# kabachuha/sd-webui-text2video

Measured on AMD Instinct MI355X. Metric: denoised frames/sec (UNet+VAE), ModelScope 24f@256x256, higher is better.
Workload: dtype f16; 1 GPU; ModelScope t2v fp16 (random-init 1.41B UNetSD + VAE decoder), 24 frames @ 256x256, 50 DDIM_Gaussian steps, CFG 9.0 (BASELINE.json configs[1]); one step = one whole video; frames_per_video=24, videos_per_batch=1, layout=single, layout_requested=auto, parallelism=1 GPU: cond+uncond batched as b=2

## Files before the change

include/t2v_hip.h:

```cpp
#ifndef T2V_HIP_H
#define T2V_HIP_H

#include <stdint.h>

#ifdef __cplusplus
extern "C" {
#endif

#define T2V_ABI_VERSION 11

#define T2V_OK 0
#define T2V_ERR_BAD_ARG (-1)
#define T2V_ERR_UNSUPPORTED (-2)
#define T2V_ERR_LAUNCH (-3)
#define T2V_ERR_NO_DEVICE (-4)
#define T2V_ERR_COMM (-5)
#define T2V_ERR_ASYNC (-6)
#define T2V_ERR_RESIDENCY (-7)

#define T2V_RELPOS_MAX_FRAMES 1024
#define T2V_RELPOS_LONG_PADL 72
#define T2V_RELPOS_LONG_COLS(R) ((2 * (R) + 158) / 8 * 8)

enum t2v_op_kind {
// ... 26 lines not shown
enum t2v_gather {
  T2V_GATHER_PLAIN = 0,
  T2V_GATHER_CONV3X3 = 1,
  T2V_GATHER_TCONV3 = 2,
  T2V_GATHER_CONV3X3_C8 = 3
};

#define T2V_EPI_NONE 0
#define T2V_EPI_GEGLU 1
#define T2V_EPI_TATTN 2

#define T2V_EPI_STATS 3

#define T2V_EPI_GN 4
#define T2V_EPI_XATTN 5
#define T2V_GN_PIECES 36

#define T2V_F16 0
#define T2V_F32 1

#define T2V_EXT_SLOTS 16
#define T2V_EXT_X 1
#define T2V_EXT_T 2
#define T2V_EXT_CTX 3
#define T2V_EXT_OUT 4
#define T2V_EXT_XT 5
#define T2V_EXT_XT_OUT 6
#define T2V_EXT_NOISE 7
#define T2V_EXT_EPS 8
#define T2V_EXT_ADAPTER 9
// ... 60 lines not shown
```

sd-webui-text2video_amd/_lib.py:

```python
from __future__ import annotations

import ctypes
import os

_HERE = os.path.dirname(os.path.abspath(__file__))
LIB_PATH = os.environ.get("T2V_LIB_PATH") or os.path.join(_HERE, "libt2v_hip.so")

EXPERIMENTAL = os.environ.get("T2V_EXPERIMENTAL", "0") == "1"


def knob(name: str, default):
    if os.environ.get("T2V_EXPERIMENTAL", "0") == "1":
        return os.environ.get(name, default)
    return default


ABI_VERSION = 11
RELPOS_MAX_FRAMES = 1024
RELPOS_LONG_PADL = 72
OP_GEMM, OP_GROUPNORM, OP_LAYERNORM, OP_ATTENTION, OP_SOFTMAX = 1, 2, 3, 4, 5
OP_NCTHW_TO_CL, OP_CL_TO_NCTHW, OP_TIME_EMBED, OP_COPY2D, OP_DDIM_STEP, OP_MEMSET = 6, 7, 8, 9, 10, 11
OP_LINCOMB = 12
OP_RELPOS_ATTN = 13
OP_EMBED_ROWS = 14
OP_TO_UINT8, OP_ALLGATHER, OP_HALO_EXCHANGE = 15, 16, 17
OP_RESHARD_ROWS, OP_ALLTOALL, OP_STATS_HALO = 18, 19, 20
OP_RESAMPLE = 21
OP_DEPTH_TOKENS, OP_AVGPOOL2 = 22, 23
ACT_NONE, ACT_SILU, ACT_RELU = 0, 1, 2
GATHER_PLAIN, GATHER_CONV3X3, GATHER_TCONV3, GATHER_CONV3X3_C8 = 0, 1, 2, 3
EPI_NONE, EPI_GEGLU, EPI_TATTN, EPI_STATS, EPI_GN, EPI_XATTN = 0, 1, 2, 3, 4, 5
GN_PIECES = 36
F16, F32 = 0, 1
EXT_SLOTS = 16
EXT_X, EXT_T, EXT_CTX, EXT_OUT, EXT_XT, EXT_XT_OUT, EXT_NOISE, EXT_EPS = 1, 2, 3, 4, 5, 6, 7, 8
EXT_ADAPTER = 9
OP_NI, OP_NF, OP_NP = 32, 8, 12
GN_ROWS_PER_BLOCK = 64
SYNC_INTS = 4096
SYNC_BARRIER_INTS = 512
GN_PART_BYTES = 2 << 20

EXPORTS = [
    "t2v_abi_version", "t2v_last_error", "t2v_device_info", "t2v_run_ops", "t2v_plan_create",
    "t2v_plan_num_ops", "t2v_plan_run", "t2v_plan_run_timed", "t2v_plan_destroy",
    "t2v_unet_forward", "t2v_vae_decode", "t2v_ddim_step",
# ... 93 lines not shown
```

sd-webui-text2video_amd/csrc/executor.hip:

```cpp
#include <hip/hip_runtime.h>

#include <cstdio>
#include <cstring>
#include <string>
#include <vector>

#include "t2v_kernels.h"

namespace {

thread_local std::string g_err;

int fail(int code, const std::string& msg) {
  g_err = msg;
  return code;
}

struct Resolved {
  t2v_op op;
};

inline bool resolve_ptrs(t2v_op& op, const uint64_t* ext, int n_ext) {
  for (int k = 0; k < T2V_OP_NP; ++k) {
    const uint64_t v = op.p[k];
// ... 24 lines not shown
      } else if (g == T2V_GATHER_CONV3X3_C8) {
        if (op.i[10] != 8 || K != 72 || op.i[3] != 8) return bad("C8 conv needs Cin == lda == 8, K == 72");
      } else if (g != T2V_GATHER_PLAIN) {
        return bad("unknown gather mode");
      }
      if (g == T2V_GATHER_CONV3X3 || g == T2V_GATHER_CONV3X3_C8) {
        if (op.i[11] != 1 && op.i[11] != 2) return bad("stride must be 1 or 2");
        if (op.i[12] != 0 && op.i[12] != 1) return bad("upsample must be 0 or 1");
        if (op.i[13] <= 0 || op.i[14] <= 0 || M % (op.i[13] * op.i[14]) != 0) return bad("M not a multiple of Hout*Wout");
      }
      if (g == T2V_GATHER_TCONV3 && (op.i[8] <= 0 || op.i[9] <= 0 || M % (op.i[8] * op.i[9]) != 0))
        return bad("M not a multiple of F*HW");
      if (op.i[16] == T2V_EPI_GEGLU && (N % 32 != 0 || op.i[17] != T2V_F16)) return bad("GEGLU needs N % 32 == 0, fp16 out");
      if (op.i[16] == T2V_EPI_STATS && (op.p[7] == 0 || op.i[19] > 1 || (g == T2V_GATHER_PLAIN && op.i[8] == 1)))
        return bad("column statistics (T2V_EPI_STATS): strips pointer p[7], no split-K, no fused LayerNorm");
      if (op.i[16] < 0 || op.i[16] > T2V_EPI_XATTN) return bad("unknown epilogue");
      if (op.i[18] < 0 || op.i[18] > 2) return bad("unknown activation (0 none, 1 SiLU, 2 ReLU)");
      if (op.i[30] != 0) {
        if (op.i[30] < 0 || M > 2 * op.i[30] || op.p[4] == 0) return bad("residual row wrap i[30]: positive, M <= 2 * wrap, and a residual");
        if (op.i[16] == T2V_EPI_GEGLU || op.i[16] == T2V_EPI_TATTN || op.i[16] == T2V_EPI_XATTN || (g == T2V_GATHER_PLAIN && (op.i[12] != 0 || op.i[8] != 0)))
          return bad("residual row wrap i[30]: plain / statistics / GroupNorm epilogues only, not beside i[12] or a fused LayerNorm");
      }
      if (op.i[16] == T2V_EPI_XATTN) {
        const int tile = op.i[22];
        if (g != T2V_GATHER_PLAIN || N % 64 != 0 || K % 64 != 0 || op.i[17] != T2V_F16 || op.i[19] > 1 || op.i[18] != 0 || op.i[8] != 0 || op.i[11] == 1)
          return bad("fused cross-attention: plain gather, N = 64 * heads, K % 64 == 0, fp16 out, no split-K / activation / LayerNorm / hi + lo output");
        if (!(((tile == 8 || tile == 11) && N == 320) || ((tile == 0 || tile == 5) && N % 128 == 0))) return bad("fused cross-attention: tile 8 / 11 with N == 320, or tile 0 / 5 with N % 128 == 0");
        if (op.p[2] != 0 || op.p[3] != 0 || op.p[4] != 0 || op.p[8] == 0 || op.p[9] == 0 || !(op.f[1] > 0.f)) return bad("fused cross-attention: no bias / row bias / residual; K, V^T and a positive scale are required");
        if (op.i[25] < 1 || op.i[25] > 96 || op.i[24] < N || op.i[24] % 8 != 0 || op.i[26] < ((op.i[25] + 31) / 32) * 32 || op.i[26] % 8 != 0 || op.i[15] <= 0 || op.i[15] % 32 != 0 || op.i[27] < 0 || op.i[28] < 0)
          return bad("fused cross-attention: 1 .. 96 keys, ld(K) >= N, V^T rows of >= ceil32(keys) halfs, rows per sample a multiple of 32");
        if (op.i[5] < N || op.i[5] % 4 != 0) return bad("fused cross-attention: ldc");
        if (op.i[12] != 0) return bad("fused cross-attention: no residual wrap");
        return 0;
      }
      if (op.i[16] == T2V_EPI_GN) {
        const int tile = op.i[22], rows = op.i[24], groups = op.i[28];
        const int bm = tile == 8 ? 192 : 128, bn = (tile == 8 || tile == 11) ? 320 : (tile == 3 ? 256 : 128);
        if (g == T2V_GATHER_CONV3X3_C8 || (g == T2V_GATHER_CONV3X3 && op.i[12] != 0)) return bad("fused GroupNorm: not for the C8 stem / the upsampling gather");
        if (op.i[20] != 0 || K % 64 != 0 || op.i[18] != 0) return bad("fused GroupNorm: no bias along M, no activation, K % 64 == 0");
        if (g == T2V_GATHER_PLAIN && (op.i[8] != 0 || op.i[11] == 1)) return bad("fused GroupNorm: no fused LayerNorm / hi + lo output on the same op");
        if (groups <= 0 || N % groups != 0 || rows <= 0 || M % rows != 0) return bad("fused GroupNorm: N % groups == 0, rows per instance must divide M");
        if (op.i[19] > 1) {
          if (groups > 32 || N % 8 != 0 || N / 8 > 512 || op.p[6] == 0) return bad("fused GroupNorm on a split-K GEMM: groups <= 32, N % 8 == 0, N <= 4096, a slab workspace");
        } else {
          if (tile != 8 && tile != 11 && tile != 3 && tile != 5 && tile != 0) return bad("fused GroupNorm: tile must be 8, 11, 3, 5 or 0");
          if (tile == 0 && N % 128 != 0) return bad("fused GroupNorm on the 128x128-class kernel: N % 128 == 0");
          if (N / groups > bn || (bn + N / groups - 1) / (N / groups) + 1 > T2V_GN_PIECES) return bad("fused GroupNorm: a group no wider than the tile");
// ... 237 lines not shown
      p.res = reinterpret_cast<const float*>(op.p[4]);
      p.out = reinterpret_cast<void*>(op.p[5]);
      p.ws = reinterpret_cast<float*>(op.p[6]);
      p.halo = op.i[23];
      p.out_lo = (p.gather == T2V_GATHER_PLAIN && op.i[11] == 1) ? 1 : 0;
      if (p.gather == T2V_GATHER_PLAIN && op.i[16] != T2V_EPI_TATTN) { p.res_wrap = op.i[12]; p.a_wrap = op.i[13]; }
      if (op.i[30] > 0) p.res_wrap = op.i[30];
      const int tile = op.i[22];
      if (p.epi == T2V_EPI_TATTN) {
        p.F = op.i[8]; p.HW = op.i[9]; p.tpix = op.i[10];
        p.tiles_ps = (p.HW + p.tpix - 1) / p.tpix;
        p.attn_scale_log2 = op.f[1] * 1.44269504088896340736f;
        p.Hin = p.Win = 0; p.Cin = 0;
        return t2v_launch_gemm2(p, tile, s);
      }
      if (p.epi == T2V_EPI_XATTN) {
        p.epi = T2V_EPI_NONE;
        p.xa_k = reinterpret_cast<const f16*>(op.p[8]);
        p.xa_vt = reinterpret_cast<const f16*>(op.p[9]);
        p.xa_ldk = op.i[24]; p.xa_lc = op.i[25]; p.xa_lcp = op.i[26]; p.xa_k_sample = op.i[27]; p.xa_vt_sample = op.i[28];
        p.attn_scale_log2 = op.f[1] * 1.44269504088896340736f;
      }
      const bool ln_any = p.gather == T2V_GATHER_PLAIN && (op.i[8] == 1 || op.i[8] == 2);
      if (p.splitk > 1 && !ln_any) p.tickets = reinterpret_cast<int*>(op.p[7]);
      if (ln_any) {
        p.ln_gb = reinterpret_cast<const float*>(op.p[3]);
        p.rowbias = nullptr;
        p.ln_out = reinterpret_cast<f16*>(op.p[7]);
        p.ld_ln = op.i[9];
        p.ln_eps = op.f[0];
// ... 260 lines not shown
```

sd-webui-text2video_amd/csrc/gemm2.hip:

```cpp
#include "t2v_kernels.h"

namespace {

__device__ __attribute__((aligned(256))) unsigned char g2_zero_page[256];

constexpr int G_CONV_UP = 100;
constexpr int BM_OF(int wm, int tm) { return wm * tm * 32; }

template <int N>
__device__ __forceinline__ void wait_vmcnt() {
  asm volatile("s_waitcnt vmcnt(%0)" ::"n"(N) : "memory");
}

template <int WM, int WN, int TM, int TN, int BK, int STAGES, int MINW, int GATHER, int XE = 0, bool TAT = false>
__global__ __launch_bounds__(WM * WN * 64, MINW) void gemm2_kernel(const GemmParams p) {
  constexpr int NW = WM * WN;
  constexpr int BM = WM * TM * 32, BN = WN * TN * 32;
  constexpr int ROW_BYTES = BK * 2;
  constexpr int RPS = 1024 / ROW_BYTES;
  constexpr int CPR = BK / 8;
  constexpr int XSLABS = BM / RPS, WSLABS = BN / RPS;
  static_assert(XSLABS % NW == 0, "token slabs must divide evenly over the waves");
  constexpr int XPW = XSLABS / NW;
  constexpr int WPW = (WSLABS + NW - 1) / NW;
// ... 485 lines not shown
      else e = launch_cfg_gather<WM, WN, TM, TN, BK, STAGES, MINW, T2V_GATHER_CONV3X3>(p, s);
      break;
    case T2V_GATHER_TCONV3:
      if constexpr (GN_TILE) {
        if (gn_here) { e = launch_cfg_gather<WM, WN, TM, TN, BK, STAGES, MINW, T2V_GATHER_TCONV3, 2>(p, s); break; }
      }
      e = launch_cfg_gather<WM, WN, TM, TN, BK, STAGES, MINW, T2V_GATHER_TCONV3>(p, s);
      break;
    default: return hipErrorInvalidValue;
  }
  if (e != hipSuccess) return e;
  if (p.splitk > 1 && p.tickets == nullptr) e = p.gn_out != nullptr ? t2v_launch_splitk_reduce_gn(p, s) : t2v_launch_splitk_reduce(p, s);
  return e;
}

}

hipError_t t2v_launch_gemm2(const GemmParams& p, int tile, hipStream_t s) {
  switch (tile) {
    case 1: return launch_cfg<2, 4, 4, 2, 64, 2, 2>(p, s);
    case 2: return launch_cfg<4, 2, 2, 5, 64, 2, 2>(p, s);
    case 3: return launch_cfg<2, 4, 2, 2, 64, 3, 2>(p, s);
    case 4: return launch_cfg<2, 2, 2, 2, 64, 4, 1>(p, s);
    case 5: return launch_cfg<2, 4, 2, 1, 64, 4, 2>(p, s);
    case 8: return launch_cfg<6, 2, 1, 5, 64, 2, 3>(p, s);
    case 9: return launch_cfg<6, 2, 1, 4, 64, 2, 3>(p, s);
    case 10: return launch_cfg<6, 2, 1, 3, 64, 2, 3>(p, s);
    case 12: return launch_cfg<2, 2, 1, 1, 64, 4, 2>(p, s);
    case 11: return launch_cfg<4, 2, 1, 5, 64, 2, 2>(p, s);
    default: return hipErrorInvalidValue;
// ... 3 lines not shown
```

sd-webui-text2video_amd/csrc/t2v_kernels.h:

```cpp
#pragma once
#include <hip/hip_runtime.h>
#include <stdint.h>

#include <string>

#include "../../include/t2v_hip.h"

typedef _Float16 f16;
typedef f16 f16x4 __attribute__((ext_vector_type(4)));
typedef f16 f16x8 __attribute__((ext_vector_type(8)));
typedef float f32x4 __attribute__((ext_vector_type(4)));
typedef float f32x8 __attribute__((ext_vector_type(8)));
typedef float f32x16 __attribute__((ext_vector_type(16)));

struct GemmParams {
  const f16* A;
  const f16* W;
  const float* bias;
  const float* rowbias;
  const float* res;
  void* out;
  float* ws;
  int M, N, K;
  int m_begin;
// ... 16 lines not shown
  int out_lo;
  float* stats;
  int a_wrap, res_wrap;
  const float* gn_gb;
  f16* gn_out;
  double* gn_part;
  unsigned* gn_bar;
  unsigned* gn_fault;
  int ld_gn, gn_rows, gn_cpg, gn_silu, gn_lo, gn_store_out;
  float gn_eps;
  int ln_x;
  unsigned gn_seq, gn_want;
  const f16* xa_k;
  const f16* xa_vt;
  int xa_ldk, xa_lc, xa_lcp, xa_k_sample, xa_vt_sample;
};


#if defined(__HIP_DEVICE_COMPILE__) && !defined(__gfx950__) && !defined(__gfx942__)
#error "libt2v_hip is written for gfx950 (MI355X); the device-scope exchange helpers assume gfx94x / gfx950 memory semantics"
#endif

__device__ __forceinline__ void t2v_st_dev(float* p, f32x4 v) { asm volatile("global_store_dwordx4 %0, %1, off sc1" ::"v"(p), "v"(v) : "memory"); }
__device__ __forceinline__ f32x4 t2v_ld_dev(const float* p) {
  f32x4 v;
  asm volatile("global_load_dwordx4 %0, %1, off sc1" : "=&v"(v) : "v"(p) : "memory");
  return v;
}
__device__ __forceinline__ void t2v_wait_dev(f32x4& a, f32x4& b, f32x4& c, f32x4& d) {
  asm volatile("s_waitcnt vmcnt(0)" : "+v"(a), "+v"(b), "+v"(c), "+v"(d)::"memory");
// ... 93 lines not shown
  return hipSuccess;
}
inline long t2v_lcm(long a, long b) { long x = a, y = b; while (y) { const long t = x % y; x = y; y = t; } return a / x * b; }

inline void t2v_normalize_splitk(GemmParams& p, int bk, long tiles) {
  const int KT = (p.K + bk - 1) / bk;
  if (p.splitk > KT) p.splitk = KT;
  if (p.splitk < 1) p.splitk = 1;
  p.kt_per_split = (KT + p.splitk - 1) / p.splitk;
  p.splitk = (KT + p.kt_per_split - 1) / p.kt_per_split;
  if (p.splitk <= 1 || p.epi != T2V_EPI_NONE || tiles > T2V_SYNC_INTS || p.gn_out != nullptr) p.tickets = nullptr;
}

hipError_t t2v_launch_gemm(const GemmParams& p, hipStream_t s);
hipError_t t2v_launch_gemm2(const GemmParams& p, int tile, hipStream_t s);
hipError_t t2v_launch_splitk_reduce(const GemmParams& p, hipStream_t s);
hipError_t t2v_launch_splitk_reduce_gn(const GemmParams& p, hipStream_t s);
hipError_t t2v_launch_groupnorm(const t2v_op& op, hipStream_t s);
hipError_t t2v_launch_layernorm(const t2v_op& op, hipStream_t s);
hipError_t t2v_launch_attention(const t2v_op& op, hipStream_t s);
hipError_t t2v_launch_relpos_attention(const t2v_op& op, hipStream_t s);
hipError_t t2v_launch_softmax(const t2v_op& op, hipStream_t s);
hipError_t t2v_launch_ncthw_to_cl(const t2v_op& op, hipStream_t s);
hipError_t t2v_launch_cl_to_ncthw(const t2v_op& op, hipStream_t s);
hipError_t t2v_launch_to_uint8(const t2v_op& op, hipStream_t s);
hipError_t t2v_launch_resample(const t2v_op& op, hipStream_t s);
hipError_t t2v_launch_depth_tokens(const t2v_op& op, hipStream_t s);
hipError_t t2v_launch_avgpool2(const t2v_op& op, hipStream_t s);
hipError_t t2v_launch_reshard_rows(const t2v_op& op, hipStream_t s);
hipError_t t2v_launch_time_embed(const t2v_op& op, hipStream_t s);
// ... 889 lines not shown
```

sd-webui-text2video_amd/lowering.py:

```python
from __future__ import annotations

from typing import Callable, Dict, List, Optional, Tuple

import torch

from . import _lib as L
from . import packing as pk
from .program import Buf, Program, Ref, TShardSpec


class _Declarations:
    def __init__(self, label: str, keep_taps: bool = False):
        self.P = Program(label)
        self.P.keep_taps = keep_taps
        self.packer = pk.WeightPacker()

    def w_linear(self, key) -> Ref:
        return Ref("weight", 0, self.packer.add(key + ":lin", "f16", lambda sd, k=key: pk.pad_rows(pk.linear(sd[k + ".weight"]))))

    def conv3_kernel(self, key) -> Tuple[Callable, str]:
        return (lambda sd, k=key: sd[k + ".weight"]), ":c3"

    def w_conv3(self, key, cin_pad=0, form="") -> Ref:
        kernel, suffix = self.conv3_kernel(key)
# ... 23 lines not shown
        self.sharing = bool(getattr(net, "_share_now", False)) and B == 2 and x_batch == 1 and self.shard is None
        self.Bc = 1 if self.sharing else B
        self.x_dt, self.out_dt, self.ctx_dt = x_dt, out_dt, ctx_dt
        self.x_batch = x_batch if 0 < x_batch < B else 0
        self.precise = bool(getattr(net, "precise_operands", False))
        level = getattr(net, "precise_operands", False)
        self.precise_gn = self.precise and level != "r3"
        self.precise_ff = self.precise and level != "r3"
        self.precise_all_levels = level == "all"
        self.precise_attn = self.precise and bool(getattr(net, "precise_attn_out", False))
        self.precise_rs = self.precise and bool(getattr(net, "precise_resample", False))
        self.gn_strips = bool(getattr(net, "gn_producer_stats", False))
        self.last_stats: Optional[Buf] = None
        self.stem_dup = False
        self.P.small_rank_tiles = self.shard is not None
        prefixes = tuple(getattr(net, "split_weight_prefixes", ()) or ())
        if prefixes:
            self.P.weight_lo = lambda ref: (Ref("weight", 0, self.packer.add_lo(ref.name))
                                            if ref.name.startswith(prefixes) and ref.name.rsplit(":", 1)[-1] in ("lin", "lin2", "c3", "c3d", "t3", "qkv", "kv")
                                            else None)
        self.emb_slices: Dict[str, Tuple[int, int]] = {}
        self.kv_slices: Dict[str, Tuple[int, int]] = {}
        self.kv_all: Optional[Buf] = None

    def precise_at(self, flag: bool, h: int, w: int) -> bool:
        return bool(flag) and (self.precise_all_levels or (h == self.H and w == self.W))

    def w_proj(self, key, copies: int) -> Ref:
        assert copies in (1, 2)
        return self.w_linear(key) if copies == 1 else self.w_linear_dup(key)

# ... 150 lines not shown
        if parting:
            self.sharing, self.Bc = False, self.B
        a = P.alloc(self.Bc * F * hw, out_cols or inner, "f16")
        lo = a.ld
        if q is None and not self.to_q_attention(attn, nrm, a, inner, heads, hw, scale, shared_rows):
            q = P.alloc(Mq, inner, "f16")
            P.gemm(attn + ".to_q", nrm, self.w_linear(attn + ".to_q"), inner, inner, q)
        if q is not None:
            P.attention(attn, q.ref, kbuf.ref, vbuf.ref, a.ref, out_buf=a, nq=hw, nk=Lc, heads=heads,
                        b_outer=self.Bc, b_inner=F, q_strides=(inner, q_b_stride, hw * inner),
                        kv_strides=(kv.ld, Lc * kv.ld, 0), o_strides=(lo, F * hw * lo, hw * lo), scale=scale, **attn_kw)
            P.free(q)
        P.free(nrm)
        return a, shared_rows

    def ff_tail(self, tb, n: Buf, x3: Buf, inner, h, w) -> Buf:
        P, M = self.P, n.rows
        wg, bg = self.w_geglu(f"{tb}.ff.net.0.proj")
        g = P.alloc(M, 4 * inner, "f16")
        P.gemm(f"{tb}.ff.geglu", n, wg, 8 * inner, inner, g, bias=bg, epi=L.EPI_GEGLU)
        P.free(n)
        hilo = self.precise_at(self.precise_ff, h, w)
        x4 = P.alloc(M, 2 * inner if hilo else inner, "f16")
        P.gemm(f"{tb}.ff.net.2", g, self.w_linear(f"{tb}.ff.net.2"), inner, 4 * inner, x4.col_slice(0, inner) if hilo else x4,
               bias=self.vec(f"{tb}.ff.net.2.bias"), residual=x3, out_lo=hilo)
        P.free(g, x3)
        return x4

    def resample(self, prefix, attr, x: Buf, c, h, w, *, up, dest: Optional[Buf] = None, **conv_kw) -> Buf:
        hilo = bool(self.precise_rs and c % 64 == 0)
        x16 = self.operand16(prefix + ".cast", x, c, hilo)
        out = self.conv3(f"{prefix}.{attr}", x16, f"{prefix}.{attr}", c, h, w, stride=1 if up else 2, up=1 if up else 0, dest=dest, hilo=hilo,
                         **conv_kw)
# ... 141 lines not shown
```

sd-webui-text2video_amd/program.py:

```python
from __future__ import annotations

import ctypes
import math
import os
from dataclasses import dataclass, field
from typing import Dict, List, Optional, Tuple

from . import _lib as L

_ITEM = {"f16": 2, "f32": 4, "f64": 8, "u8": 1}
COLLECTIVE_KINDS = (L.OP_ALLGATHER, L.OP_HALO_EXCHANGE, L.OP_ALLTOALL, L.OP_STATS_HALO)
_DT = {"f16": L.F16, "f32": L.F32}


@dataclass(frozen=True)
class TShardSpec:
    size: int
    index: int
    counts: Tuple[int, ...]

    @staticmethod
    def make(total_frames: int, size: int, index: int) -> "TShardSpec":
        base = -(-total_frames // size)
        last = total_frames - base * (size - 1)
# ... 78 lines not shown
                    self.free_list[idx] = (off + n, size - n)
                self.live[off] = n
                return off
        if self.free_list and self.free_list[-1][0] + self.free_list[-1][1] == self.top:
            off, size = self.free_list.pop()
            self.top = off
        off = self.top
        self.top += n
        self.high = max(self.high, self.top)
        self.live[off] = n
        return off

    def free(self, off: int):
        n = self.live.pop(off)
        self.free_list.append((off, n))
        self.free_list.sort()
        merged: List[Tuple[int, int]] = []
        for o, s in self.free_list:
            if merged and merged[-1][0] + merged[-1][1] == o:
                merged[-1] = (merged[-1][0], merged[-1][1] + s)
            else:
                merged.append((o, s))
        self.free_list = merged


@dataclass
class Op:
    kind: int
    name: str
    i: List[int] = field(default_factory=lambda: [0] * L.OP_NI)
    f: List[float] = field(default_factory=lambda: [0.0] * L.OP_NF)
    p: List[Ref] = field(default_factory=lambda: [NULL] * L.OP_NP)
    flops: float = 0.0
    meta: dict = field(default_factory=dict)
    out: Optional["Buf"] = None
    out2: Optional["Buf"] = None


# ... 9 lines not shown
        self.small_rank_tiles = False
        self.gn_fused_slice_bytes = int(L.knob("T2V_GN_FUSED_SLICE", 64 * 1024))
        self.gn_fused_total_bytes = int(L.knob("T2V_GN_FUSED_TOTAL", 128 * 1024 * 1024))
        self.weight_lo = None
        self._sync: Buf = self.alloc(L.SYNC_INTS + L.SYNC_BARRIER_INTS, 1, "f32")
        self.splitk_tickets = L.knob("T2V_SPLITK_TICKETS", "0") != "0"
        self.gn_coop = os.environ.get("T2V_GN_COOP", "1") != "0"
        self.gn_epilogue = self.gn_coop and os.environ.get("T2V_GN_EPI", "1") != "0" and not L.exchange_disabled()
        self._gn_part: Optional[Buf] = self.alloc(L.GN_PART_BYTES, 1, "u8") if self.gn_epilogue else None
        self._deferred: List[Buf] = []

    def alloc(self, rows: int, cols: int, dtype: str, ld: Optional[int] = None) -> Buf:
        ld = cols if ld is None else ld
        off = self.arena.alloc(rows * ld * _ITEM[dtype])
        return Buf(Ref("arena", off), rows, cols, ld, dtype, off)

    def free(self, *bufs: Buf):
        for b in bufs:
            if b is None or b.alloc_off < 0 or not b.owns:
                continue
            if self.keep_taps and any(t.alloc_off == b.alloc_off for t in self.taps.values()):
                continue
            if self._is_operand_of_last_gemm(b):
                self._deferred.append(b)
                continue
            self.arena.free(b.alloc_off)

    def _is_operand_of_last_gemm(self, b: Buf) -> bool:
        if not getattr(self, "gn_epilogue", False) or not self.ops:
            return False
# ... 267 lines not shown
                       stats=int(with_stats))
        if ln_fused:
            op.out2 = ln[3]
        if step_invariant:
            op.meta["step_invariant"] = True
        self._emit(op)
        if ln is not None and not ln_fused:
            self.layernorm(name + ".ln", out if m is None else out.row_slice(0, M), gamma, beta,
                           ln_out if m is None else ln_out.row_slice(0, M), ln_eps)
        if ws is not None:
            self.free(ws)
        if lo_tmp is not None:
            self.free(lo_tmp)
        return op

    def to_q_cross_attention(self, name: str, a: Buf, w: Ref, out: Buf, *, k: int, heads: int, kbuf: Buf, vt: Buf, n_keys: int,
                             rows_per_sample: int, samples: int, scale: float, a_wrap: int = 0) -> Optional[Op]:
        n = heads * 64
        M = out.rows
        assert a.dtype == "f16" and out.dtype == "f16" and out.cols == n and k % 64 == 0 and n_keys <= 96 and rows_per_sample % 32 == 0
        tile, split = self.choose_tile(M, n, k, L.GATHER_PLAIN, allow_splitk=False)
        if not (((tile in (8, 11)) and n == 320) or (tile in (0, 5) and n % 128 == 0)) or split != 1:
            return None
        op = Op(L.OP_GEMM, name)
        I = op.i
        I[0], I[1], I[2] = M, n, k
        I[3], I[4], I[5] = a.ld, k, out.ld
        I[7], I[13], I[15] = L.GATHER_PLAIN, a_wrap, rows_per_sample
        I[16], I[17], I[19], I[22] = L.EPI_XATTN, L.F16, 1, tile
        I[24], I[25], I[26], I[27], I[28] = kbuf.ld, n_keys, vt.ld, n_keys * kbuf.ld, vt.rows // samples * vt.ld
# ... 567 lines not shown
```

sd-webui-text2video_amd/unet.py:

```python
from __future__ import annotations

import os
from functools import partial
from typing import Dict, Optional, Tuple

import numpy as np
import torch
import torch.nn as nn

from . import _lib as L
from . import packing as pk
from .lowering import _UNetLowering
from .program import COLLECTIVE_KINDS, BoundProgram, Buf, Program, Ref


def unet_layout(dim, dim_mult, num_res_blocks, attn_scales, temporal_attention=True):
    enc = [dim * u for u in [1] + list(dim_mult)]
    dec = [dim * u for u in [dim_mult[-1]] + list(dim_mult[::-1])]
    shortcut = [dim]
    scale = 1.0
    inputs, middle, outputs = [], [], []
    stem = [("stem", None, dim)] + ([("tt", dim, dim)] if temporal_attention else [])
    inputs.append(("input_blocks.0", stem, False))
    idx = 1
# ... 163 lines not shown
        self.debug_taps = False
        self.norm_input_dtype = L.knob("T2V_NORM_INPUT", "f16")
        self.gn_producer_stats = L.knob("T2V_GN_STRIPS", "0") != "0"
        self.context_token = None
        self.single_timestep = False
        self._share_now = False
        self.split_weight_prefixes = ()
        self.precise_operands = {"0": False, "r3": "r3", "all": "all"}.get(os.environ.get("T2V_PRECISE", "1"), True)
        self.precise_attn_out = L.knob("T2V_PRECISE_ATTN", "0") != "0"
        self.precise_resample = L.knob("T2V_PRECISE_RESAMPLE", "0") != "0"
        self.fused_temporal_attention = {"0": False, "force": "force"}.get(L.knob("T2V_FUSED_TATTN", "1"), True)
        self.t_shard = None
        self.eps_out_dtype = None
        self.share_cfg_prefix = L.knob("T2V_SHARE_PREFIX", "1") != "0"
        self.fused_cross_attention = L.knob("T2V_XATTN", "0") != "0"
        self.auto_refresh = True
        self.device = torch.device("cpu")

    def _make(self, kind, cin, cout, dropout, decoder, stem=False):
        if kind == "stem":
            return nn.Conv2d(self.in_dim, cout, 3, padding=1)
        if kind == "res":
            return _res_block_params(cin, self.embed_dim, cout, dropout)
        if kind == "st":
            return _spatial_transformer_params(cout, cout // self.head_dim, self.head_dim,
                                               1024 if decoder else self.context_dim)
        if kind == "tt":
            heads = self.num_heads if stem else cout // self.head_dim
            return _temporal_transformer_params(cout, heads, self.head_dim)
        if kind == "down":
# ... 163 lines not shown
            comp.bound.run(ext, torch.cuda.current_stream(x.device).cuda_stream, skip_invariant=reuse)
        else:
            comp.bound.run(ext, torch.cuda.current_stream(x.device).cuda_stream)
        comp.ctx_token, comp.ctx_bound = token, comp.bound
        return out

    def _program_key(self, B, F, H, W, Lctx, x_dtype, y_dtype, out_dtype, shard=None, Bx=None):
        return (B, F, H, W, Lctx, _dt(x_dtype), _dt(y_dtype), _dt(out_dtype)) + ((shard,) if shard else ()) + \
            ((("xb", Bx),) if (Bx is not None and Bx != B) else ()) + \
            ((("split",) + tuple(self.split_weight_prefixes),) if self.split_weight_prefixes else ()) + self._lowering_options()

    def _lowering_options(self) -> tuple:
        return ((("strips",),) if getattr(self, "gn_producer_stats", False) else ()) + \
            ((("share",),) if getattr(self, "_share_now", False) else ()) + \
            ((("xattn",),) if getattr(self, "fused_cross_attention", False) else ()) + \
            ((("pattn",),) if (getattr(self, "precise_attn_out", False) and type(self) is not UNetSD) else ()) + ((("presample",),) if getattr(self, "precise_resample", False) else ()) + \
            ((("precise", str(self.precise_operands)),) if getattr(self, "precise_operands", False) else ()) + \
            ((("tattn", str(self.fused_temporal_attention)),) if getattr(self, "fused_temporal_attention", False) else ())

    def forward_cfg_pair(self, x, t, ctx_pair, context_token=None, single_t=None):
        tt = t.to(device=x.device, dtype=torch.float32).reshape(-1)
        if single_t is None:
            single_t = tt.shape[0] == 1 or bool((tt == tt[0]).all())
        tt = tt.repeat(ctx_pair.shape[0] // tt.shape[0]) if tt.shape[0] != ctx_pair.shape[0] else tt
        self.context_token = context_token
        self.single_timestep = bool(single_t)
        return UNetSD.forward(self, x, tt, ctx_pair)

    max_programs = 4

# ... 333 lines not shown
```

sd-webui-text2video_amd/videocrafter.py:

```python
from __future__ import annotations

import math
from functools import partial
from typing import List, Optional

import numpy as np
import torch
import torch.nn as nn

from . import _lib as L
from . import packing as pk
from .program import Buf, Program, Ref
from .lowering import _UNetLowering
from .unet import UNetSD, _Compiled, _attn_params


def lvdm_layout(model_channels, channel_mult, num_res_blocks, attention_resolutions):
    mc = model_channels
    inputs = [("input_blocks.0", [("stem", None, mc)])]
    chans = [mc]
    ch, ds, idx = mc, 1, 1
    for level, mult in enumerate(channel_mult):
        for _ in range(num_res_blocks):
            parts = [("res", ch, mult * mc)]
# ... 214 lines not shown

    def _compile(self, B, F, H, W, Lctx, x_dt, out_dt, ctx_dt="f32", shard=None, x_batch=0, adapter=None):
        low = _LvdmLowering(self, B, F, H, W, Lctx, x_dt, out_dt, ctx_dt, keep_taps=self.debug_taps, shard=shard, x_batch=x_batch,
                            adapter=adapter or 0)
        return _Compiled(low.build(), low.packer)


class _LvdmLowering(_UNetLowering):
    head_per_frame = False

    def __init__(self, *args, adapter: int = 0, **kwargs):
        super().__init__(*args, **kwargs)
        self.adapter_fb = int(adapter)
        self.n_feat = 0
        assert not self.adapter_fb or self.shard is None, "adapter features are not sharded along T"

    def conv3_kernel(self, key):
        return (lambda sd, k=key: sd[k + ".weight"][:, :, 0]), ":c133"

    def table(self, key) -> Ref:
        return Ref("weight", 0, self.packer.add(key + ":tab", "f32", lambda sd, k=key: sd[k]))

    def table16(self, key, frames: int, transposed: bool) -> Optional[Ref]:
        if frames > 16 or self.net.temporal_length < frames - 1:
            return None
        return Ref("weight", 0, self.packer.add(f"{key}:tab16{'T' if transposed else ''}.{frames}", "f16",
                                                lambda sd, k=key, f=frames, t=transposed: pk.relpos_table16(sd[k].float(), f, t)))

    def table_long(self, key, frames: int, transposed: bool) -> Optional[Ref]:
        if frames <= 32 and str(L.knob("T2V_RELPOS_MFMA", "2")) != "3":
# ... 755 lines not shown
```

Baseline: 17.98 frames/s.

## Fuse GEGLU feed-forward into a single kernel keeping the hidden activation in LDS

Adds a fused feed-forward kernel for inner width 320. Each 192-row block computes the GEGLU projection one 64-wide hidden slice at a time, applies bias and erf-GELU gating into LDS, and accumulates the second projection in registers through a 3-stage global-to-LDS ring. This is meant to avoid writing and re-reading the M x 1280 hidden tensor and to save a kernel launch per transformer block at high-resolution levels (M >= 24576). It is enabled by default for the UNet and adds arena placement logic for the output buffer. The risk is that the large per-block LDS footprint and 12-wave blocks lower occupancy compared with the two tuned GEMMs.

Result: no change. 18.06 frames/s, median of 6 (+0.5%).

```diff
diff --git a/include/t2v_hip.h b/include/t2v_hip.h
--- a/include/t2v_hip.h
+++ b/include/t2v_hip.h
@@ -64,6 +64,7 @@
 
 #define T2V_EPI_GN 4
 #define T2V_EPI_XATTN 5
+#define T2V_EPI_FF 6
 #define T2V_GN_PIECES 36
 
 #define T2V_F16 0
diff --git a/sd-webui-text2video_amd/_lib.py b/sd-webui-text2video_amd/_lib.py
--- a/sd-webui-text2video_amd/_lib.py
+++ b/sd-webui-text2video_amd/_lib.py
@@ -29,7 +29,7 @@
 OP_DEPTH_TOKENS, OP_AVGPOOL2 = 22, 23
 ACT_NONE, ACT_SILU, ACT_RELU = 0, 1, 2
 GATHER_PLAIN, GATHER_CONV3X3, GATHER_TCONV3, GATHER_CONV3X3_C8 = 0, 1, 2, 3
-EPI_NONE, EPI_GEGLU, EPI_TATTN, EPI_STATS, EPI_GN, EPI_XATTN = 0, 1, 2, 3, 4, 5
+EPI_NONE, EPI_GEGLU, EPI_TATTN, EPI_STATS, EPI_GN, EPI_XATTN, EPI_FF = 0, 1, 2, 3, 4, 5, 6
 GN_PIECES = 36
 F16, F32 = 0, 1
 EXT_SLOTS = 16
diff --git a/sd-webui-text2video_amd/csrc/executor.hip b/sd-webui-text2video_amd/csrc/executor.hip
--- a/sd-webui-text2video_amd/csrc/executor.hip
+++ b/sd-webui-text2video_amd/csrc/executor.hip
@@ -62,11 +62,11 @@
       if (op.i[16] == T2V_EPI_GEGLU && (N % 32 != 0 || op.i[17] != T2V_F16)) return bad("GEGLU needs N % 32 == 0, fp16 out");
       if (op.i[16] == T2V_EPI_STATS && (op.p[7] == 0 || op.i[19] > 1 || (g == T2V_GATHER_PLAIN && op.i[8] == 1)))
         return bad("column statistics (T2V_EPI_STATS): strips pointer p[7], no split-K, no fused LayerNorm");
-      if (op.i[16] < 0 || op.i[16] > T2V_EPI_XATTN) return bad("unknown epilogue");
+      if (op.i[16] < 0 || op.i[16] > T2V_EPI_FF) return bad("unknown epilogue");
       if (op.i[18] < 0 || op.i[18] > 2) return bad("unknown activation (0 none, 1 SiLU, 2 ReLU)");
       if (op.i[30] != 0) {
         if (op.i[30] < 0 || M > 2 * op.i[30] || op.p[4] == 0) return bad("residual row wrap i[30]: positive, M <= 2 * wrap, and a residual");
-        if (op.i[16] == T2V_EPI_GEGLU || op.i[16] == T2V_EPI_TATTN || op.i[16] == T2V_EPI_XATTN || (g == T2V_GATHER_PLAIN && (op.i[12] != 0 || op.i[8] != 0)))
+        if (op.i[16] == T2V_EPI_GEGLU || op.i[16] == T2V_EPI_TATTN || op.i[16] == T2V_EPI_XATTN || op.i[16] == T2V_EPI_FF || (g == T2V_GATHER_PLAIN && (op.i[12] != 0 || op.i[8] != 0)))
           return bad("residual row wrap i[30]: plain / statistics / GroupNorm epilogues only, not beside i[12] or a fused LayerNorm");
       }
       if (op.i[16] == T2V_EPI_XATTN) {
@@ -79,6 +79,17 @@
           return bad("fused cross-attention: 1 .. 96 keys, ld(K) >= N, V^T rows of >= ceil32(keys) halfs, rows per sample a multiple of 32");
         if (op.i[5] < N || op.i[5] % 4 != 0) return bad("fused cross-attention: ldc");
         if (op.i[12] != 0) return bad("fused cross-attention: no residual wrap");
+        return 0;
+      }
+      if (op.i[16] == T2V_EPI_FF) {
+        const int hidden = op.i[24];
+        if (g != T2V_GATHER_PLAIN || N != 320 || K != 320 || op.i[19] > 1 || op.i[17] != T2V_F16 || op.i[18] != 0 || op.i[20] != 0 || op.i[8] != 0 || op.i[22] != 8)
+          return bad("fused feed-forward: plain gather, N == 320, K == 320, tile 8, fp16 out, no split-K / activation / fused LayerNorm");
+        if (hidden < 64 || hidden > 1280 || hidden % 64 != 0 || op.i[25] < hidden || op.i[25] % 8 != 0 || op.i[4] < K) return bad("fused feed-forward: hidden i[24] a multiple of 64 in 64 .. 1280, ld(W2) i[25] >= hidden and a multiple of 8, ldw >= K");
+        if (op.i[12] != 0 || op.i[13] != 0 || op.p[3] != 0 || op.p[6] != 0 || op.p[7] != 0) return bad("fused feed-forward: no row wrap, row bias, split-K workspace or statistics");
+        if (op.p[0] == 0 || op.p[1] == 0 || op.p[5] == 0 || op.p[8] == 0) return bad("fused feed-forward: A, W1, out and W2 are required");
+        if (op.i[11] != 0 && op.i[11] != 1) return bad("fused feed-forward: i[11] is the hi + lo output flag (0 | 1)");
+        if (op.i[5] < N * (op.i[11] == 1 ? 2 : 1) || (op.p[4] != 0 && (op.i[6] < N || op.i[6] % 4 != 0))) return bad("fused feed-forward: ldc >= N (2 N with the hi + lo output), ldr >= N and a multiple of 4");
         return 0;
       }
       if (op.i[16] == T2V_EPI_GN) {
@@ -346,6 +357,16 @@
         p.Hin = p.Win = 0; p.Cin = 0;
         return t2v_launch_gemm2(p, tile, s);
       }
+      if (p.epi == T2V_EPI_FF) {
+        p.epi = T2V_EPI_NONE;
+        p.ff_b1 = p.bias;
+        p.bias = reinterpret_cast<const float*>(op.p[9]);
+        p.ff_w2 = reinterpret_cast<const f16*>(op.p[8]);
+        p.ff_hidden = op.i[24]; p.ff_ldw2 = op.i[25];
+        p.rowbias = nullptr; p.ws = nullptr; p.res_wrap = p.a_wrap = 0;
+        p.Hin = p.Win = 0; p.Cin = 0;
+        return t2v_launch_ff_fused(p, s);
+      }
       if (p.epi == T2V_EPI_XATTN) {
         p.epi = T2V_EPI_NONE;
         p.xa_k = reinterpret_cast<const f16*>(op.p[8]);
diff --git a/sd-webui-text2video_amd/csrc/gemm2.hip b/sd-webui-text2video_amd/csrc/gemm2.hip
--- a/sd-webui-text2video_amd/csrc/gemm2.hip
+++ b/sd-webui-text2video_amd/csrc/gemm2.hip
@@ -523,6 +523,184 @@
   return e;
 }
 
+constexpr int FF_BM = 192, FF_NW = 12, FF_STAGES = 3, FF_LPS = 4;
+constexpr int FF_STAGE_BYTES = 40 * 1024, FF_A_BYTES = 24 * 1024, FF_H_BYTES = 24 * 1024;
+constexpr int FF_OFF_H = FF_STAGES * FF_STAGE_BYTES;
+constexpr int FF_OFF_DUMMY = FF_OFF_H + FF_H_BYTES;
+constexpr int FF_OFF_B1 = FF_OFF_DUMMY + 1024;
+constexpr int FF_MAX_HIDDEN = 1280;
+constexpr int FF_LDS_MAX = FF_OFF_B1 + 2 * FF_MAX_HIDDEN * 4;
+static_assert(FF_LDS_MAX + 64 <= 160 * 1024, "the fused feed-forward must fit one CU's LDS");
+static_assert(FF_NW * 32 * T2V_EPI_SP * 4 <= FF_OFF_H, "the row-coalescing buffers of the tail re-use the ring");
+
+__global__ __launch_bounds__(FF_NW * 64, 3) void ff_fused_kernel(const GemmParams p) {
+  extern __shared__ __attribute__((aligned(16))) unsigned char smem[];
+  const int tid = threadIdx.x;
+  const int lane = tid & 63;
+  const int wave = __builtin_amdgcn_readfirstlane(tid >> 6);
+  const int wm = wave >> 1, wn = wave & 1;
+  const int m0 = blockIdx.x * FF_BM;
+  const int nslices = p.ff_hidden >> 6;
+  const unsigned char* zero = g2_zero_page;
+
+  {
+    float* b1s = reinterpret_cast<float*>(smem + FF_OFF_B1);
+    for (int i = tid * 4; i < 2 * p.ff_hidden; i += FF_NW * 64 * 4) {
+      f32x4 v = {0.f, 0.f, 0.f, 0.f};
+      if (p.ff_b1) v = *reinterpret_cast<const f32x4*>(p.ff_b1 + i);
+      *reinterpret_cast<f32x4*>(b1s + i) = v;
+    }
+  }
+  __syncthreads();
+
+  const int lrow = lane >> 3, pchunk = lane & 7;
+  const int lcb = (pchunk ^ (4 * (wave & 1) + (lrow >> 1))) * 16;
+  const int prow = wave * 8 + lrow;
+  const unsigned char* abase = reinterpret_cast<const unsigned char*>(p.A + (long)(m0 + prow) * p.lda) + lcb;
+  const bool aok0 = m0 + prow < p.M, aok1 = m0 + prow + 96 < p.M;
+  const long astride = (long)96 * p.lda * 2;
+  const unsigned char* w1base = reinterpret_cast<const unsigned char*>(p.W + (size_t)prow * p.ldw) + lcb;
+  const long w1stride = (long)96 * p.ldw * 2, w1slice = (long)128 * p.ldw * 2;
+  const unsigned char* w2base = reinterpret_cast<const unsigned char*>(p.ff_w2 + (size_t)prow * p.ff_ldw2) + lcb;
+  const long w2stride = (long)96 * p.ff_ldw2 * 2;
+  const bool tail_dummy = wave >= 4;
+
+  int fs = 0, fj = 0;
+  auto fill_piece = [&](int slot, int q) {
+    unsigned char* stage = smem + slot * FF_STAGE_BYTES;
+    const unsigned char* src = zero;
+    unsigned char* dst = stage + (wave + 12 * q) * 1024;
+    const bool live = fs < nslices;
+    if (fj < 5) {
+      if (q < 2) {
+        if (live && (q == 0 ? aok0 : aok1)) src = abase + q * astride + fj * 128;
+      } else if (q == 3 && tail_dummy) {
+        dst = smem + FF_OFF_DUMMY;
+      } else {
+        if (live) src = w1base + (q - 2) * w1stride + fs * w1slice + fj * 128;
+        dst = stage + FF_A_BYTES + (wave + 12 * (q - 2)) * 1024;
+      }
+    } else {
+      if (q == 3 && tail_dummy) dst = smem + FF_OFF_DUMMY;
+      else if (live) src = w2base + q * w2stride + fs * 128;
+    }
+    t2v_glds16(src, dst);
+  };
+  auto fill_end = [&]() {
+    if (++fj == 6) { fj = 0; ++fs; }
+  };
+
+  f32x16 O[1][5], U[2];
+#pragma unroll
+  for (int b = 0; b < 5; ++b)
+#pragma unroll
+    for (int r = 0; r < 16; ++r) O[0][b][r] = 0.f;
+#pragma unroll
+  for (int b = 0; b < 2; ++b)
+#pragma unroll
+    for (int r = 0; r < 16; ++r) U[b][r] = 0.f;
+
+#pragma unroll
+  for (int g = 0; g < FF_STAGES - 1; ++g) {
+#pragma unroll
+    for (int q = 0; q < FF_LPS; ++q) fill_piece(g, q);
+    fill_end();
+  }
+
+  const int frow = lane & 31, fhalf = lane >> 5;
+  const int fsw = ((frow >> 1) & 7) << 4;
+  const int xoff = (wm * 32 + frow) * 128;
+  const int w1off = FF_A_BYTES + (wn * 64 + frow) * 128;
+  const int w2off = (wn * 160 + frow) * 128;
+  const unsigned char* Hs = smem + FF_OFF_H;
+  const float* b1s = reinterpret_cast<const float*>(smem + FF_OFF_B1);
+  const int nhalf = fhalf * 4;
+
+  int slot = 0;
+  auto step_begin = [&]() -> int {
+    asm volatile("s_waitcnt vmcnt(%0) lgkmcnt(0)" ::"n"(FF_LPS * (FF_STAGES - 2)) : "memory");
+    __builtin_amdgcn_s_barrier();
+    asm volatile("" ::: "memory");
+    int f = slot + FF_STAGES - 1;
+    return f >= FF_STAGES ? f - FF_STAGES : f;
+  };
+  auto step_end = [&]() {
+    fill_end();
+    slot = slot + 1 == FF_STAGES ? 0 : slot + 1;
+  };
+
+  for (int s = 0; s < nslices; ++s) {
+#pragma unroll 1
+    for (int kt = 0; kt < 5; ++kt) {
+      const int fslot = step_begin();
+      const unsigned char* st = smem + slot * FF_STAGE_BYTES;
+#pragma unroll
+      for (int kk = 0; kk < 4; ++kk) {
+        const int lc4 = ((kk * 2 + fhalf) << 4) ^ fsw;
+        const f16x8 xf = *reinterpret_cast<const f16x8*>(st + xoff + lc4);
+        const f16x8 wf0 = *reinterpret_cast<const f16x8*>(st + w1off + lc4);
+        const f16x8 wf1 = *reinterpret_cast<const f16x8*>(st + w1off + 4096 + lc4);
+        fill_piece(fslot, kk);
+        U[0] = __builtin_amdgcn_mfma_f32_32x32x16_f16(wf0, xf, U[0], 0, 0, 0);
+        U[1] = __builtin_amdgcn_mfma_f32_32x32x16_f16(wf1, xf, U[1], 0, 0, 0);
+      }
+      step_end();
+    }
+    {
+      unsigned char* hrow = smem + FF_OFF_H + xoff + nhalf * 2;
+#pragma unroll
+      for (int b = 0; b < 2; ++b)
+#pragma unroll
+        for (int qq = 0; qq < 2; ++qq) {
+          const int pc = s * 128 + wn * 64 + b * 32 + 16 * qq + nhalf;
+          const f32x4 bv = *reinterpret_cast<const f32x4*>(b1s + pc);
+          const f32x4 bg = *reinterpret_cast<const f32x4*>(b1s + pc + 8);
+          f16x4 o;
+#pragma unroll
+          for (int r = 0; r < 4; ++r) o[r] = (f16)((U[b][8 * qq + r] + bv[r]) * t2v_gelu_erf(U[b][8 * qq + 4 + r] + bg[r]));
+          const int chunk = wn * 4 + b * 2 + qq;
+          *reinterpret_cast<f16x4*>(hrow + ((chunk << 4) ^ fsw)) = o;
+        }
+#pragma unroll
+      for (int b = 0; b < 2; ++b)
+#pragma unroll
+        for (int r = 0; r < 16; ++r) U[b][r] = 0.f;
+    }
+    {
+      const int fslot = step_begin();
+      const unsigned char* st = smem + slot * FF_STAGE_BYTES;
+#pragma unroll
+      for (int kk = 0; kk < 4; ++kk) {
+        const int lc4 = ((kk * 2 + fhalf) << 4) ^ fsw;
+        const f16x8 xf = *reinterpret_cast<const f16x8*>(Hs + xoff + lc4);
+        f16x8 wf[5];
+#pragma unroll
+        for (int b = 0; b < 5; ++b) wf[b] = *reinterpret_cast<const f16x8*>(st + w2off + b * 4096 + lc4);
+        fill_piece(fslot, kk);
+#pragma unroll
+        for (int b = 0; b < 5; ++b) O[0][b] = __builtin_amdgcn_mfma_f32_32x32x16_f16(wf[b], xf, O[0][b], 0, 0, 0);
+      }
+      step_end();
+    }
+  }
+  wait_vmcnt<0>();
+  __builtin_amdgcn_s_barrier();
+  asm volatile("" ::: "memory");
+  t2v_epilogue_rows<1, 5>(p, O, reinterpret_cast<float*>(smem) + wave * (32 * T2V_EPI_SP), lane, m0 + wm * 32, wn * 160, 0);
+}
+
+}
+
+hipError_t t2v_launch_ff_fused(const GemmParams& p, hipStream_t s) {
+  if (p.N != 320 || p.K != 320 || p.ff_hidden < 64 || p.ff_hidden > FF_MAX_HIDDEN || p.ff_hidden % 64 != 0 || p.splitk != 1 || p.out_f32 ||
+      p.gather != T2V_GATHER_PLAIN)
+    return hipErrorInvalidValue;
+  static t2v_device_flags attr_set;
+  const hipError_t e = t2v_set_dynamic_lds(reinterpret_cast<const void*>(ff_fused_kernel), FF_LDS_MAX, attr_set, s);
+  if (e != hipSuccess) return e;
+  const int lds = FF_OFF_B1 + 2 * p.ff_hidden * 4;
+  hipLaunchKernelGGL(ff_fused_kernel, dim3((p.M + FF_BM - 1) / FF_BM), dim3(FF_NW * 64), lds, s, p);
+  return hipGetLastError();
 }
 
 hipError_t t2v_launch_gemm2(const GemmParams& p, int tile, hipStream_t s) {
diff --git a/sd-webui-text2video_amd/csrc/t2v_kernels.h b/sd-webui-text2video_amd/csrc/t2v_kernels.h
--- a/sd-webui-text2video_amd/csrc/t2v_kernels.h
+++ b/sd-webui-text2video_amd/csrc/t2v_kernels.h
@@ -54,6 +54,9 @@
   const f16* xa_k;
   const f16* xa_vt;
   int xa_ldk, xa_lc, xa_lcp, xa_k_sample, xa_vt_sample;
+  const f16* ff_w2;
+  const float* ff_b1;
+  int ff_ldw2, ff_hidden;
 };
 
 
@@ -177,6 +180,7 @@
 
 hipError_t t2v_launch_gemm(const GemmParams& p, hipStream_t s);
 hipError_t t2v_launch_gemm2(const GemmParams& p, int tile, hipStream_t s);
+hipError_t t2v_launch_ff_fused(const GemmParams& p, hipStream_t s);
 hipError_t t2v_launch_splitk_reduce(const GemmParams& p, hipStream_t s);
 hipError_t t2v_launch_splitk_reduce_gn(const GemmParams& p, hipStream_t s);
 hipError_t t2v_launch_groupnorm(const t2v_op& op, hipStream_t s);
diff --git a/sd-webui-text2video_amd/lowering.py b/sd-webui-text2video_amd/lowering.py
--- a/sd-webui-text2video_amd/lowering.py
+++ b/sd-webui-text2video_amd/lowering.py
@@ -61,7 +61,7 @@
         self.last_stats: Optional[Buf] = None
         self.stem_dup = False
         self.P.small_rank_tiles = self.shard is not None
-        prefixes = tuple(getattr(net, "split_weight_prefixes", ()) or ())
+        prefixes = self.split_prefixes = tuple(getattr(net, "split_weight_prefixes", ()) or ())
         if prefixes:
             self.P.weight_lo = lambda ref: (Ref("weight", 0, self.packer.add_lo(ref.name))
                                             if ref.name.startswith(prefixes) and ref.name.rsplit(":", 1)[-1] in ("lin", "lin2", "c3", "c3d", "t3", "qkv", "kv")
@@ -242,9 +242,22 @@
         P.free(nrm)
         return a, shared_rows
 
+    def ff_fused_here(self, tb, M: int, inner: int) -> bool:
+        mode = getattr(self.net, "ff_fuse", False)
+        if not mode or inner != 320 or (mode != "force" and M < Program.FF_FUSED_MIN_ROWS):
+            return False
+        return not (self.split_prefixes and f"{tb}.ff.net.2:lin".startswith(self.split_prefixes))
+
     def ff_tail(self, tb, n: Buf, x3: Buf, inner, h, w) -> Buf:
         P, M = self.P, n.rows
         wg, bg = self.w_geglu(f"{tb}.ff.net.0.proj")
+        if self.ff_fused_here(tb, M, inner):
+            hilo = self.precise_at(self.precise_ff, h, w)
+            x4 = P.alloc_as_behind(M, 2 * inner if hilo else inner, "f16", scratch_bytes=M * 4 * inner * 2, operand=n)
+            P.ff_fused(f"{tb}.ff.fused", n, wg, bg, self.w_linear(f"{tb}.ff.net.2"), self.vec(f"{tb}.ff.net.2.bias"),
+                       x4.col_slice(0, inner) if hilo else x4, hidden=4 * inner, residual=x3, out_lo=hilo)
+            P.free(n, x3)
+            return x4
         g = P.alloc(M, 4 * inner, "f16")
         P.gemm(f"{tb}.ff.geglu", n, wg, 8 * inner, inner, g, bias=bg, epi=L.EPI_GEGLU)
         P.free(n)
diff --git a/sd-webui-text2video_amd/program.py b/sd-webui-text2video_amd/program.py
--- a/sd-webui-text2video_amd/program.py
+++ b/sd-webui-text2video_amd/program.py
@@ -116,6 +116,9 @@
     def free(self, off: int):
         n = self.live.pop(off)
         self.free_list.append((off, n))
+        self._coalesce()
+
+    def _coalesce(self):
         self.free_list.sort()
         merged: List[Tuple[int, int]] = []
         for o, s in self.free_list:
@@ -124,6 +127,28 @@
             else:
                 merged.append((o, s))
         self.free_list = merged
+
+    def alloc_at(self, off: int, nbytes: int) -> int:
+        n = (max(nbytes, 1) + self.ALIGN - 1) // self.ALIGN * self.ALIGN
+        end = off + n
+        assert off % self.ALIGN == 0
+        if end > self.top:
+            self.free_list.append((self.top, end - self.top))
+            self.top = end
+            self.high = max(self.high, end)
+            self._coalesce()
+        for idx, (o, s) in enumerate(self.free_list):
+            if o <= off and end <= o + s:
+                self.free_list[idx:idx + 1] = ([(o, off - o)] if off > o else []) + ([(end, o + s - end)] if o + s > end else [])
+                self.live[off] = n
+                return off
+        raise ValueError(f"arena range [{off}, {end}) is not free")
+
+    def snapshot(self):
+        return list(self.free_list), self.top, dict(self.live), self.high
+
+    def restore(self, snap):
+        self.free_list, self.top, self.live, self.high = list(snap[0]), snap[1], dict(snap[2]), snap[3]
 
 
 @dataclass
@@ -163,6 +188,26 @@
         ld = cols if ld is None else ld
         off = self.arena.alloc(rows * ld * _ITEM[dtype])
         return Buf(Ref("arena", off), rows, cols, ld, dtype, off)
+
+    def alloc_as_behind(self, rows: int, cols: int, dtype: str, *, scratch_bytes: int, operand: Buf) -> Buf:
+        A, nbytes = self.arena, rows * cols * _ITEM[dtype]
+        assert operand.owns and operand.alloc_off in A.live
+        snap = A.snapshot()
+        A.alloc(scratch_bytes)
+        for b in self._deferred:
+            if b.alloc_off in A.live:
+                A.free(b.alloc_off)
+        lo, hi = operand.alloc_off, operand.alloc_off + A.live[operand.alloc_off]
+        A.free(operand.alloc_off)
+        off = A.alloc(nbytes)
+        size = A.live[off]
+        A.restore(snap)
+        self._flush_deferred()
+        if off + size <= lo or off >= hi:
+            A.alloc_at(off, nbytes)
+        else:
+            off = A.alloc(nbytes)
+        return Buf(Ref("arena", off), rows, cols, cols, dtype, off)
 
     def free(self, *bufs: Buf):
         for b in bufs:
@@ -460,6 +505,31 @@
             self.free(lo_tmp)
         return op
 
+    FF_FUSED_MIN_ROWS = 24576
+
+    def ff_fused(self, name: str, a: Buf, w1: Ref, b1: Ref, w2: Ref, b2: Ref, out: Buf, *, hidden: int, residual: Optional[Buf] = None,
+                 out_lo: bool = False) -> Op:
+        M, n, k = out.rows, 320, 320
+        assert a.dtype == "f16" and a.cols == k and a.rows >= M and out.dtype == "f16" and out.cols == n
+        assert hidden % 64 == 0 and 64 <= hidden <= 1280
+        assert not out_lo or out.ld >= 2 * n
+        op = Op(L.OP_GEMM, name)
+        I = op.i
+        I[0], I[1], I[2] = M, n, k
+        I[3], I[4], I[5] = a.ld, k, out.ld
+        I[6] = residual.ld if residual is not None else 0
+        I[7], I[11] = L.GATHER_PLAIN, 1 if out_lo else 0
+        I[16], I[17], I[19], I[22] = L.EPI_FF, L.F16, 1, 8
+        I[24], I[25] = hidden, hidden
+        if residual is not None:
+            assert residual.dtype == "f32" and residual.rows >= M and residual.cols == n
+        op.p[0], op.p[1], op.p[2], op.p[5], op.p[8], op.p[9] = a.ref, w1, b1, out.ref, w2, b2
+        op.p[4] = residual.ref if residual is not None else NULL
+        op.flops = 2.0 * M * (2 * hidden) * k + 2.0 * M * n * hidden
+        op.out = out
+        op.meta = dict(M=M, N=n, K=k, gather=L.GATHER_PLAIN, conv={}, epi=L.EPI_FF, split=1, tile=8, halo=False, ln=0, hidden=hidden)
+        return self._emit(op)
+
     def to_q_cross_attention(self, name: str, a: Buf, w: Ref, out: Buf, *, k: int, heads: int, kbuf: Buf, vt: Buf, n_keys: int,
                              rows_per_sample: int, samples: int, scale: float, a_wrap: int = 0) -> Optional[Op]:
         n = heads * 64
diff --git a/sd-webui-text2video_amd/unet.py b/sd-webui-text2video_amd/unet.py
--- a/sd-webui-text2video_amd/unet.py
+++ b/sd-webui-text2video_amd/unet.py
@@ -201,6 +201,7 @@
         self.eps_out_dtype = None
         self.share_cfg_prefix = L.knob("T2V_SHARE_PREFIX", "1") != "0"
         self.fused_cross_attention = L.knob("T2V_XATTN", "0") != "0"
+        self.ff_fuse = {"0": False, "force": "force"}.get(L.knob("T2V_FF_FUSE", "1"), True)
         self.auto_refresh = True
         self.device = torch.device("cpu")
 
@@ -394,6 +395,7 @@
         return ((("strips",),) if getattr(self, "gn_producer_stats", False) else ()) + \
             ((("share",),) if getattr(self, "_share_now", False) else ()) + \
             ((("xattn",),) if getattr(self, "fused_cross_attention", False) else ()) + \
+            ((("ff", str(self.ff_fuse)),) if getattr(self, "ff_fuse", False) else ()) + \
             ((("pattn",),) if (getattr(self, "precise_attn_out", False) and type(self) is not UNetSD) else ()) + ((("presample",),) if getattr(self, "precise_resample", False) else ()) + \
             ((("precise", str(self.precise_operands)),) if getattr(self, "precise_operands", False) else ()) + \
             ((("tattn", str(self.fused_temporal_attention)),) if getattr(self, "fused_temporal_attention", False) else ())
diff --git a/sd-webui-text2video_amd/videocrafter.py b/sd-webui-text2video_amd/videocrafter.py
--- a/sd-webui-text2video_amd/videocrafter.py
+++ b/sd-webui-text2video_amd/videocrafter.py
@@ -252,6 +252,9 @@
         self.adapter_fb = int(adapter)
         self.n_feat = 0
         assert not self.adapter_fb or self.shard is None, "adapter features are not sharded along T"
+
+    def ff_fused_here(self, tb, M: int, inner: int) -> bool:
+        return getattr(self.net, "ff_fuse", False) == "force" and super().ff_fused_here(tb, M, inner)
 
     def conv3_kernel(self, key):
         return (lambda sd, k=key: sd[k + ".weight"][:, :, 0]), ":c133"
```
